# eceo-epfl/ScaleProtoSeg

Measured on AMD Instinct MI355X. Metric: Mpix/s fwd+bwd prototype-distance, Cityscapes 1024x2048, higher is better.
Workload: dtype bf16; 1 GPU; cityscapes_1024x2048_c256_p190_s1; latent_px_per_gpu=2097152, channels=256, prototypes=190, scales=1, classes=19, features_dtype=bf16, parallelism=single

## Files before the change

include/spx_hip.h:

```cpp
#ifndef SPX_HIP_H
#define SPX_HIP_H

#include <stddef.h>
#include <stdint.h>

#ifdef __cplusplus
extern "C" {
#endif

#define SPX_MAX_PANELS 64
#define SPX_ABI_VERSION 17
#define SPX_PRUNE_MAX_K 64

typedef struct spx_plan {
    int32_t num_prototypes;
    int32_t num_classes;
    int32_t num_scales;
    int32_t channels_per_scale;
    int32_t kc;
    int32_t npb;
    int32_t ncb;
    int32_t npanels;
    int32_t panel_ch0[SPX_MAX_PANELS];
    int32_t panel_p0[SPX_MAX_PANELS];
// ... 83 lines not shown
               float* d_logits, void* stream);
int spx_ce_finish(const float* partials, int64_t n_pairs, float* loss, float* count_sum, void* stream);
int spx_shift_labels(const void* labels, int32_t is_int64, int64_t n, int32_t* out, void* stream);

size_t spx_pixel_outer_workspace_bytes(int64_t M, int32_t n1, int32_t n2);
int spx_pixel_outer(const float* a, const float* b, int64_t M, int32_t n1, int32_t n2, float* out, void* workspace, void* stream);

size_t spx_rows_gemm_workspace_bytes(int32_t M, int32_t N, int32_t K, int32_t flags);
int spx_rows_gemm(const float* A, int64_t a_row_stride, int64_t a_k_stride, const float* B, int64_t b_row_stride,
                  int64_t b_k_stride, float* C, int64_t ldc, int32_t M, int32_t N, int32_t K, int32_t flags, const float* E,
                  int64_t lde, void* workspace, void* stream);

size_t spx_group_tail_workspace_bytes(const spx_plan* plan, int32_t B, int32_t HW);
int spx_dist_fwd_group_ws(const spx_plan* plan, const void* x, int32_t x_dtype, int32_t B, int32_t HW,
                          const void* packed_bank, const float* packed_p2, const void* packed_head,
                          const float* Wg, int32_t K2, float* distances, float* activations,
                          float* group_activations, float* logits, const spx_ce* ce, void* workspace,
                          float epsilon, int32_t act_fn, void* stream);
int spx_dist_bwd_group_ce(const spx_plan* plan, const void* x, int32_t x_dtype, int32_t B, int32_t HW,
                          const void* packed_bank, const void* packed_bankT, const float* packed_p2,
                          const void* packed_headT_units, const void* packed_tailT, int32_t K2,
                          const float* group_activations, const float* d_dist, const float* d_act,
                          const spx_ce* ce, const float* d_group_activations, float* d_units, void* dx, void* dx_acc, void* g_out,
                          void* a_out, float epsilon, int32_t act_fn, void* stream);

int spx_group_dense(const float* const* block_ptrs, const int32_t* block_cols, int32_t nblocks, const int32_t* row_block,
                    const int32_t* row_local, const int32_t* col_block, const int32_t* col_local, int32_t U, int32_t P, float* out,
                    void* stream);
int spx_group_dense_bwd(const float* d_out, const int32_t* flat_row, const int32_t* flat_col, int64_t n, int32_t P, float* d_flat,
                        void* stream);
size_t spx_packed_tail_bytes(const spx_plan* plan);
int spx_pack_group_tail(const spx_plan* plan, const float* Wg, int32_t K2, void* packed_tail, void* packed_tailT,
                        void* stream);
int spx_pack_headT_units(const spx_plan* plan, const float* W, void* packed_headT_units, void* stream);
int spx_dist_fwd_group(const spx_plan* plan, const void* x, int32_t x_dtype, int32_t B, int32_t HW,
                       const void* packed_bank, const float* packed_p2, const void* packed_head,
                       const void* packed_tail, int32_t K2,
                       float* distances, float* activations, float* group_activations, float* logits,
                       float epsilon, int32_t act_fn, void* stream);
int spx_dist_bwd_group(const spx_plan* plan, const void* x, int32_t x_dtype, int32_t B, int32_t HW,
                       const void* packed_bank, const void* packed_bankT, const float* packed_p2,
                       const void* packed_headT_units, const void* packed_tailT, int32_t K2,
                       const float* group_activations, const float* d_dist, const float* d_act,
                       const float* d_logits, const float* d_group_activations, float* d_units, void* dx, void* dx_acc, void* g_out,
                       void* a_out, float epsilon, int32_t act_fn, void* stream);
int spx_exp(const float* x, float* y, int64_t n, void* stream);
int spx_exp_bwd(const float* g, const float* y, float* dx, int64_t n, void* stream);

size_t spx_bwd_scratch_bytes(const spx_plan* plan, int32_t B, int32_t HW);
size_t spx_bwd_head_scratch_bytes(const spx_plan* plan, int32_t B, int32_t HW);
size_t spx_bwd_dx_scratch_bytes(const spx_plan* plan, int32_t x_dtype, int32_t B, int32_t HW);

size_t spx_bank_bwd_workspace_bytes(const spx_plan* plan, int32_t B, int32_t HW);
int spx_bank_bwd(const spx_plan* plan, const void* x, int32_t x_dtype, int32_t B, int32_t HW,
                 const float* bank, const void* g_in, const void* a_in, const float* d_logits,
                 float* d_bank, float* d_W, void* workspace, void* stream);

int spx_push_argmin(const float* distances, const int32_t* labels, const float* class_identity,
                    int32_t B, int32_t P, int32_t K, int32_t HW, int32_t void_class, float max_dist,
                    int64_t* indices, float* values, uint64_t* scratch, void* stream);

int spx_dist_push_min(const spx_plan* plan, const void* x, int32_t x_dtype, int32_t B, int32_t HW, const void* packed_bank,
                      const float* packed_p2, const int32_t* labels, int32_t void_class, int32_t K, const uint32_t* proto_key,
                      float max_dist, int64_t* indices, float* values, uint64_t* scratch, void* stream);

int spx_argmin_images(const float* values, int32_t N, int32_t P, int64_t* best, void* stream);

int spx_kld_segment_max(const float* vals, const int32_t* labels, int32_t B, int32_t J, int32_t HW, int32_t W, int32_t K,
                        uint32_t* smax_keys, uint32_t* counts, uint32_t* range_keys, void* stream);
int spx_kld_segment_sumexp(const float* vals, const int32_t* labels, int32_t B, int32_t J, int32_t HW, int32_t W, int32_t K,
                           const uint32_t* smax_keys, uint64_t* ssum_fx, void* stream);
int spx_kld_segment_lse(const uint32_t* smax_keys, const uint64_t* ssum_fx, int32_t n, float* lse, const uint32_t* range_keys,
                        int32_t HW, double* scale, void* stream);
int spx_kld_gram_loss(const int64_t* a_fx, const double* scale, const uint32_t* counts, const uint8_t* pair_ok, int32_t nseg, int32_t K,
                      int32_t J, float* A, float* Cf, double* partials, float* loss, void* stream);
int spx_kld_pair_sums(const float* vals, const int32_t* labels, int32_t B, int32_t J, int32_t HW, int32_t W, int32_t K,
                      const float* lse, const double* scale, int64_t* a_fx, void* stream);
int spx_kld_backward(const float* vals, const int32_t* labels, int32_t B, int32_t J, int32_t HW, int32_t K,
                     const float* lse, const float* A, const float* Cf, const float* cf_scale, float* grad, void* stream);

int spx_upsample_argext(const float* src, int32_t N, int32_t C, int32_t h, int32_t w, int32_t H, int32_t W,
                        int32_t take_max, int64_t* indices, float* values, void* stream);

int spx_eval_accumulate(const float* logits, const int64_t* host_logit_strides, const float* distances,
                        const int64_t* host_dist_strides, const int32_t* proto_class, const void* labels, int32_t label_bytes,
                        int32_t N, int32_t K, int32_t P, int32_t h, int32_t w, int32_t H, int32_t W, int64_t* conf,
                        int64_t* hits, void* stream);
int spx_eval_topk(const float* logits, const int64_t* host_logit_strides, const float* distances, const int64_t* host_dist_strides,
                  const int32_t* proto_class, const void* samples, int32_t sample_bytes, int32_t N, int32_t S, int32_t K,
                  int32_t P, int32_t h, int32_t w, int32_t H, int32_t W, int64_t* topk, int64_t* seen, void* stream);
int spx_eval_check_classes(const int32_t* host_classes, int32_t P, int32_t K);

int spx_prune_argmin(const float* distances, const int32_t* labels, int32_t void_label, int32_t B, int32_t P, int32_t HW,
                     uint64_t* keys, void* stream);
int spx_dist_prune_min(const spx_plan* plan, const void* x, int32_t x_dtype, int32_t B, int32_t HW, const void* packed_bank,
                       const float* packed_p2, const int32_t* labels, int32_t void_label, const uint32_t* proto_key, uint64_t* keys,
                       void* stream);
int spx_prune_footprint(const int32_t* labels, int32_t B, int32_t Hf, int32_t Wf, int32_t H, int32_t W, int32_t P,
                        const uint64_t* keys, const int32_t* target_class, int32_t* label, int32_t* box, void* stream);
int spx_prune_merge(const uint64_t* keys, const int32_t* label, const int32_t* box, int32_t B, int32_t P, int32_t W, int64_t image0,
                    int32_t k, uint64_t* table_key, int64_t* table_image, int32_t* table_label, int32_t* table_box, int32_t* table_cell,
                    void* stream);

#define SPX_REG_ENT 1
#define SPX_REG_CEG 2
#define SPX_REG_SMAX 4
// ... 60 lines not shown
```

scaleprotoseg_amd/_lib.py:

```python
from __future__ import annotations

import ctypes as C
import os
from typing import Optional

import torch

_HERE = os.path.dirname(os.path.abspath(__file__))
LIB_PATH = os.path.join(_HERE, "libspx_hip.so")
SPX_MAX_PANELS = 64
ABI_VERSION = 17


class SpxError(RuntimeError):
    """A libspx_hip.so entry point returned a non-zero status."""


class SpxPlan(C.Structure):
    _fields_ = [
        ("num_prototypes", C.c_int32),
        ("num_classes", C.c_int32),
        ("num_scales", C.c_int32),
        ("channels_per_scale", C.c_int32),
        ("kc", C.c_int32),
# ... 51 lines not shown
    _fields_ = [
        ("vals", C.c_void_p),
        ("labels", C.c_void_p),
        ("slot_scale", C.c_void_p),
        ("B", C.c_int32),
        ("J", C.c_int32),
        ("HW", C.c_int32),
        ("W", C.c_int32),
        ("K", C.c_int32),
        ("mode", C.c_int32),
        ("terms", C.c_int32),
        ("norm_type", C.c_int32),
        ("epsilon", C.c_float),
        ("weights", C.c_float * 3),
    ]


_PP = C.POINTER(SpxPlan)
_PCE = C.POINTER(SpxCe)
_PR = C.POINTER(SpxReg)
_PA = C.POINTER(SpxActLoss)
_V = C.c_void_p
_I = C.c_int32
_F = C.c_float
_PL = C.POINTER(C.c_int64)

SIGNATURES = {
    "spx_version": (C.c_int, []),
    "spx_last_error": (C.c_char_p, []),
    "spx_make_plan": (C.c_int, [_I, _I, _I, _I, C.POINTER(_I), C.POINTER(_I), _PP]),
    "spx_packed_bank_bytes": (C.c_size_t, [_PP]),
    "spx_packed_bankT_bytes": (C.c_size_t, [_PP]),
    "spx_packed_p2_bytes": (C.c_size_t, [_PP]),
    "spx_packed_head_bytes": (C.c_size_t, [_PP]),
    "spx_packed_headT_bytes": (C.c_size_t, [_PP]),
    "spx_pack_bank": (C.c_int, [_PP, _V, _V, _V, _V, _V]),
    "spx_pack_head": (C.c_int, [_PP, _V, _V, _V, _V]),
    "spx_pack_all": (C.c_int, [_PP, _V, _V, _V, _I, _V, _V, _V, _V, _V, _V, _V, _V]),
    "spx_dist_fwd": (C.c_int, [_PP, _V, _I, _I, _I, _V, _V, _V, _V, _V, _V, _F, _I, _V]),
    "spx_dist_bwd": (C.c_int, [_PP, _V, _I, _I, _I, _V, _V, _V, _V, _V, _V, _V, _V, _V, _V, _V, _F, _I, _V]),
    "spx_dist_fwd_cls": (C.c_int, [_PP, _V, _I, _I, _I, _V, _V, _V, _V, _V, _I, _V, _V, _V, _F, _I, _V]),
    "spx_dist_bwd_cls": (C.c_int, [_PP, _V, _I, _I, _I, _V, _V, _V, _V, _V, _V, _I, _V, _V, _V, _V, _V, _V, _V, _F, _I, _V]),
    "spx_group_dense": (C.c_int, [_V, _V, _I, _V, _V, _V, _V, _I, _I, _V, _V]),
    "spx_group_dense_bwd": (C.c_int, [_V, _V, _V, C.c_int64, _I, _V, _V]),
    "spx_packed_tail_bytes": (C.c_size_t, [_PP]),
    "spx_pack_group_tail": (C.c_int, [_PP, _V, _I, _V, _V, _V]),
    "spx_pack_headT_units": (C.c_int, [_PP, _V, _V, _V]),
    "spx_dist_fwd_group": (C.c_int, [_PP, _V, _I, _I, _I, _V, _V, _V, _V, _I, _V, _V, _V, _V, _F, _I, _V]),
    "spx_dist_bwd_group": (C.c_int, [_PP, _V, _I, _I, _I, _V, _V, _V, _V, _V, _I, _V, _V, _V, _V, _V, _V, _V, _V, _V, _V, _F, _I, _V]),
    "spx_bwd_scratch_bytes": (C.c_size_t, [_PP, _I, _I]),
    "spx_bwd_head_scratch_bytes": (C.c_size_t, [_PP, _I, _I]),
    "spx_bwd_dx_scratch_bytes": (C.c_size_t, [_PP, _I, _I, _I]),
    "spx_bank_bwd_workspace_bytes": (C.c_size_t, [_PP, _I, _I]),
    "spx_bank_bwd": (C.c_int, [_PP, _V, _I, _I, _I, _V, _V, _V, _V, _V, _V, _V, _V]),
    "spx_push_argmin": (C.c_int, [_V, _V, _V, _I, _I, _I, _I, _I, _F, _V, _V, _V, _V]),
    "spx_dist_push_min": (C.c_int, [_PP, _V, _I, _I, _I, _V, _V, _V, _I, _I, _V, _F, _V, _V, _V, _V]),
    "spx_argmin_images": (C.c_int, [_V, _I, _I, _V, _V]),
    "spx_kld_segment_max": (C.c_int, [_V, _V, _I, _I, _I, _I, _I, _V, _V, _V, _V]),
    "spx_kld_segment_sumexp": (C.c_int, [_V, _V, _I, _I, _I, _I, _I, _V, _V, _V]),
    "spx_kld_segment_lse": (C.c_int, [_V, _V, _I, _V, _V, _I, _V, _V]),
    "spx_kld_gram_loss": (C.c_int, [_V, _V, _V, _V, _I, _I, _I, _V, _V, _V, _V, _V]),
    "spx_kld_pair_sums": (C.c_int, [_V, _V, _I, _I, _I, _I, _I, _V, _V, _V, _V]),
    "spx_kld_backward": (C.c_int, [_V, _V, _I, _I, _I, _I, _V, _V, _V, _V, _V, _V]),
    "spx_upsample_argext": (C.c_int, [_V, _I, _I, _I, _I, _I, _I, _I, _V, _V, _V]),
    "spx_fwd_split_groups": (C.c_int32, [_PP, _I, _I]),
    "spx_fwd_split_workspace_bytes": (C.c_size_t, [_PP, _I, _I]),
    "spx_dist_fwd_ws": (C.c_int, [_PP, _V, _I, _I, _I, _V, _V, _V, _V, _V, _I, _V, _V, _V, _V, _V, _F, _I, _V]),
    "spx_group_tail_workspace_bytes": (C.c_size_t, [_PP, _I, _I]),
    "spx_dist_fwd_group_ws": (C.c_int, [_PP, _V, _I, _I, _I, _V, _V, _V, _V, _I, _V, _V, _V, _V, _PCE, _V, _F, _I, _V]),
    "spx_dist_bwd_group_ce": (C.c_int, [_PP, _V, _I, _I, _I, _V, _V, _V, _V, _V, _I, _V, _V, _V, _PCE, _V, _V, _V, _V, _V, _V, _F, _I, _V]),
    "spx_exp": (C.c_int, [_V, _V, C.c_int64, _V]),
    "spx_exp_bwd": (C.c_int, [_V, _V, _V, C.c_int64, _V]),
    "spx_pixel_outer_workspace_bytes": (C.c_size_t, [C.c_int64, _I, _I]),
    "spx_pixel_outer": (C.c_int, [_V, _V, C.c_int64, _I, _I, _V, _V, _V]),
    "spx_rows_gemm_workspace_bytes": (C.c_size_t, [_I, _I, _I, _I]),
    "spx_rows_gemm": (C.c_int, [_V, C.c_int64, C.c_int64, _V, C.c_int64, C.c_int64, _V, C.c_int64, _I, _I, _I, _I, _V, C.c_int64, _V, _V]),
    "spx_ce_partials": (C.c_size_t, [_I, _I]),
    "spx_ce_partials_flat": (C.c_size_t, [C.c_int64]),
    "spx_ce_finish": (C.c_int, [_V, C.c_int64, _V, _V, _V]),
    "spx_shift_labels": (C.c_int, [_V, _I, C.c_int64, _V, _V]),
    "spx_dist_fwd_ce": (C.c_int, [_PP, _V, _I, _I, _I, _V, _V, _V, _V, _V, _I, _V, _V, _V, _V, _PCE, _F, _I, _V]),
    "spx_dist_bwd_ce": (C.c_int, [_PP, _V, _I, _I, _I, _V, _V, _V, _V, _V, _V, _I, _V, _V, _V, _PCE, _V, _V, _V, _V, _F, _I, _V]),
    "spx_ce_fwd": (C.c_int, [_V, _V, C.c_int64, _I, _V, _V, _V, _V]),
    "spx_ce_bwd": (C.c_int, [_V, _V, _V, _V, C.c_int64, _I, _V, _V]),
    "spx_eval_accumulate": (C.c_int, [_V, _PL, _V, _PL, _V, _V, _I, _I, _I, _I, _I, _I, _I, _I, _V, _V, _V]),
    "spx_eval_topk": (C.c_int, [_V, _PL, _V, _PL, _V, _V, _I, _I, _I, _I, _I, _I, _I, _I, _I, _V, _V, _V]),
    "spx_eval_check_classes": (C.c_int, [C.POINTER(_I), _I, _I]),
    "spx_prune_argmin": (C.c_int, [_V, _V, _I, _I, _I, _I, _V, _V]),
    "spx_dist_prune_min": (C.c_int, [_PP, _V, _I, _I, _I, _V, _V, _V, _I, _V, _V, _V]),
    "spx_prune_footprint": (C.c_int, [_V, _I, _I, _I, _I, _I, _I, _V, _V, _V, _V, _V]),
    "spx_prune_merge": (C.c_int, [_V, _V, _V, _I, _I, _I, C.c_int64, _I, _V, _V, _V, _V, _V, _V]),
    "spx_reg_workspace_bytes": (C.c_size_t, [_PR]),
    "spx_reg_fwd": (C.c_int, [_PR, _V, _V, _V, _V]),
    "spx_reg_bwd": (C.c_int, [_PR, _V, _V, _V, _V, _V]),
    "spx_actloss_workspace_bytes": (C.c_size_t, [_PA]),
    "spx_actloss_segment_max": (C.c_int, [_PA, _V, _V]),
    "spx_actloss_segment_sums": (C.c_int, [_PA, _V, _V]),
    "spx_actloss_finish": (C.c_int, [_PA, _V, _V, _V, _V]),
    "spx_actloss_backward": (C.c_int, [_PA, _V, _V, _V, _V, _V]),
    "spx_overlap_workspace_bytes": (C.c_size_t, [_I, _I, _I]),
    "spx_overlap_thresholds": (C.c_int, [_V, _PL, _I, _I, _I, _I, _I, _I, C.c_int64, _F, _V, _V, _V]),
    "spx_overlap_accumulate": (C.c_int, [_V, _PL, _V, _V, _I, _V, _I, _I, _I, _I, _I, _I, _I, _I, _V, _V, _V, _V, _V]),
    "spx_push_boxes": (C.c_int, [_V, _PL, _V, _I, _V, _V, _V, _I, _I, _I, _I, _I, _I, _I, _I, _V, _V, _V]),
    "spx_push_merge": (C.c_int, [_V, _V, _V, _I, _I, _I, _I, _I, _I, _V, C.c_int64, _V, _V, _V, _V, _V]),
}

# ... 59 lines not shown
```

scaleprotoseg_amd/csrc/spx_api.hip:

```cpp
#include <stdarg.h>
#include <stdio.h>
#include <string.h>

#include "spx_args.h"

static thread_local char g_err[512] = "";
#ifdef SPX_DIAG
static unsigned long long* g_dbg = nullptr;
static int g_tile_mul_req = 0;
#else
static constexpr unsigned long long* g_dbg = nullptr;
static constexpr int g_tile_mul_req = 0;
#endif

static int gcd_i(int a, int b) { while (b) { const int t = a % b; a = b; b = t; } return a; }
int spx_tile_mul(int tiles_launch, long long plane_bytes) {
    int m = g_tile_mul_req;
    if (m == 0) m = (plane_bytes > 0 && plane_bytes % (1ll << 20) == 0) ? 257 : 1;
    if (m <= 1 || tiles_launch < 4 * m) return 1;
    while (gcd_i(m, tiles_launch) != 1) ++m;
    return m;
}

static int fail(const char* fmt, ...) {
// ... 520 lines not shown
    if (!g || !y || !dx || n < 1 || (n + 255) / 256 > 0x7fffffffLL) return fail("spx_exp_bwd: bad arguments");
    return hip_status(spx_launch_exp(nullptr, g, y, dx, n, (hipStream_t)stream), "spx_exp_bwd");
}

int spx_group_dense(const float* const* block_ptrs, const int32_t* block_cols, int32_t nblocks, const int32_t* row_block,
                    const int32_t* row_local, const int32_t* col_block, const int32_t* col_local, int32_t U, int32_t P, float* out,
                    void* stream) {
    if (!block_ptrs || !block_cols || !row_block || !row_local || !col_block || !col_local || !out) return fail("spx_group_dense: NULL buffer");
    if (nblocks < 1 || nblocks > SPX_GROUP_BLOCKS_MAX) return fail("spx_group_dense: %d blocks (1..%d)", nblocks, SPX_GROUP_BLOCKS_MAX);
    if (U < 1 || P < 1 || (long long)U * P > 0x7fffffffLL) return fail("spx_group_dense: bad sizes (U=%d P=%d)", U, P);
    SpxGroupDenseArgs a{};
    for (int j = 0; j < nblocks; ++j) {
        if (!block_ptrs[j] || block_cols[j] < 1) return fail("spx_group_dense: block %d is empty", j);
        a.ptrs[j] = block_ptrs[j];
        a.ncols[j] = block_cols[j];
    }
    a.row_block = row_block; a.row_local = row_local; a.col_block = col_block; a.col_local = col_local;
    a.U = U; a.P = P; a.out = out;
    return hip_status(spx_launch_group_dense(a, (hipStream_t)stream), "spx_group_dense");
}
int spx_group_dense_bwd(const float* d_out, const int32_t* flat_row, const int32_t* flat_col, int64_t n, int32_t P, float* d_flat,
                        void* stream) {
    if (!d_out || !flat_row || !flat_col || !d_flat) return fail("spx_group_dense_bwd: NULL buffer");
    if (n < 1 || P < 1 || (n + 255) / 256 > 0x7fffffffLL) return fail("spx_group_dense_bwd: bad sizes");
    return hip_status(spx_launch_group_dense_bwd(d_out, flat_row, flat_col, n, P, d_flat, (hipStream_t)stream), "spx_group_dense_bwd");
}

int spx_ce_fwd(const float* logits, const int32_t* labels, int64_t M, int32_t K, float* lse, int32_t* pred, float* partials,
               void* stream) {
    if (!logits || !labels || !lse || !partials) return fail("spx_ce_fwd: NULL buffer");
    if (M < 1 || K < 1 || (M + 255) / 256 > 0x7fffffffLL) return fail("spx_ce_fwd: bad sizes (M=%lld K=%d)", (long long)M, K);
    return hip_status(spx_launch_ce_fwd(logits, labels, M, K, lse, pred, partials, (hipStream_t)stream), "spx_ce_fwd");
}
int spx_ce_finish(const float* partials, int64_t n_pairs, float* loss, float* count_sum, void* stream) {
    if (!partials || !loss || !count_sum || n_pairs < 1) return fail("spx_ce_finish: bad arguments");
    return hip_status(spx_launch_ce_finish(partials, n_pairs, loss, count_sum, (hipStream_t)stream), "spx_ce_finish");
}
int spx_shift_labels(const void* labels, int32_t is_int64, int64_t n, int32_t* out, void* stream) {
    if (!labels || !out || n < 1 || (n + 255) / 256 > 0x7fffffffLL) return fail("spx_shift_labels: bad arguments");
    return hip_status(spx_launch_shift_labels(labels, is_int64, n, out, (hipStream_t)stream), "spx_shift_labels");
}
int spx_ce_bwd(const float* logits, const float* lse, const int32_t* labels, const float* coef, int64_t M, int32_t K,
               float* d_logits, void* stream) {
    if (!logits || !lse || !labels || !coef || !d_logits) return fail("spx_ce_bwd: NULL buffer");
    if (M < 1 || K < 1 || (M * K + 255) / 256 > 0x7fffffffLL) return fail("spx_ce_bwd: bad sizes (M=%lld K=%d)", (long long)M, K);
    return hip_status(spx_launch_ce_bwd(logits, lse, labels, coef, M, K, d_logits, (hipStream_t)stream), "spx_ce_bwd");
}

size_t spx_bank_bwd_workspace_bytes(const spx_plan* pl, int32_t B, int32_t HW) {
    const int nsplit = spx_bank_bwd_nsplit(*pl, B, HW);
    return spx_bank_bwd_ws_floats(*pl, nsplit) * sizeof(float);
}

int spx_bank_bwd(const spx_plan* pl, const void* x, int32_t x_dtype, int32_t B, int32_t HW, const float* bank,
                 const void* g_in, const void* a_in, const float* d_logits, float* d_bank, float* d_W,
                 void* workspace, void* stream) {
    if (check_plan(pl)) return 1;
    if (!x || !bank || !workspace) return fail("spx_bank_bwd: NULL operand");
    if (x_dtype != 0 && x_dtype != 1) return fail("spx_bank_bwd: x_dtype %d", x_dtype);
    if (d_bank && !g_in) return fail("spx_bank_bwd: d_bank requested without G");
    if (d_W && !a_in) return fail("spx_bank_bwd: d_W requested without the head-gradient scratch of spx_dist_bwd");
    if (d_W && pl->ncb > 1 && !d_logits) return fail("spx_bank_bwd: d_W of a head wider than 32 rows needs d_logits");
    if (pl->channels_per_scale > 256) return fail("spx_bank_bwd: Cs %d > 256 not supported", pl->channels_per_scale);
    SpxBankBwdArgs a;
    a.plan = *pl;
    a.x = x;
    a.bank = bank;
    a.g_in = (const uint16_t*)g_in;
    a.a_in = (const uint16_t*)a_in;
    a.d_logits = d_logits;
    a.d_bank = d_bank;
    a.d_W = d_W;
    a.workspace = (float*)workspace;
    a.B = B;
    a.HW = HW;
    a.nsplit = spx_bank_bwd_nsplit(*pl, B, HW);
    return hip_status(spx_launch_bank_bwd(a, x_dtype, (hipStream_t)stream), "spx_bank_bwd");
}

int spx_push_argmin(const float* distances, const int32_t* labels, const float* class_identity, int32_t B, int32_t P,
                    int32_t K, int32_t HW, int32_t void_class, float max_dist, int64_t* indices, float* values,
                    uint64_t* scratch, void* stream) {
    if (!distances || !labels || !class_identity || !indices || !values || !scratch)
        return fail("spx_push_argmin: NULL buffer");
    if (B < 1 || P < 1 || K < 1 || HW < 1) return fail("spx_push_argmin: empty input");
    if (K > 160) return fail("spx_push_argmin: num_classes %d > 160", K);
    if (P > 65535 || B > 65535) return fail("spx_push_argmin: grid too large");
    return hip_status(spx_launch_push_argmin(distances, labels, class_identity, B, P, K, HW, void_class, max_dist,
                                             indices, values, scratch, (hipStream_t)stream),
                      "spx_push_argmin");
}

int spx_prune_argmin(const float* distances, const int32_t* labels, int32_t void_label, int32_t B, int32_t P, int32_t HW,
                     uint64_t* keys, void* stream) {
    if (!distances || !labels || !keys) return fail("spx_prune_argmin: NULL buffer");
    if (B < 1 || P < 1 || HW < 1) return fail("spx_prune_argmin: empty input (B=%d P=%d HW=%d)", B, P, HW);
    if (P > 0x7FFF8 || B > 65535) return fail("spx_prune_argmin: grid too large (B=%d P=%d)", B, P);
    return hip_status(spx_launch_prune_argmin(distances, labels, void_label, B, P, HW, keys, (hipStream_t)stream), "spx_prune_argmin");
}

int spx_prune_footprint(const int32_t* labels, int32_t B, int32_t Hf, int32_t Wf, int32_t H, int32_t W, int32_t P,
                        const uint64_t* keys, const int32_t* target_class, int32_t* label, int32_t* box, void* stream) {
    if (!labels || !keys || !target_class || !label || !box) return fail("spx_prune_footprint: NULL buffer");
    if (B < 1 || P < 1 || Hf < 1 || Wf < 1 || H < 1 || W < 1)
        return fail("spx_prune_footprint: empty input (B=%d P=%d Hf=%d Wf=%d H=%d W=%d)", B, P, Hf, Wf, H, W);
    if (B > 65535 || P > 0x7FFFFFFF / 4) return fail("spx_prune_footprint: grid too large (B=%d P=%d)", B, P);
// ... 317 lines not shown
```

scaleprotoseg_amd/csrc/spx_args.h:

```cpp
#pragma once
#include "spx_common.h"
#include <type_traits>

struct SpxFwdArgs {
    spx_plan plan;
    const void* x;
    const char* packed_bank;
    const float* p2;
    const char* packed_head;
    float* dist;
    float* act;
    float* logits;
    int B, HW, vec_ok;
    int tile_first, tiles_launch;
    int tile_mul;
    int dist_vec;
    const int32_t* labels;
    const uint32_t* proto_key;
    float* cls_dist;
    int J;
    unsigned long long* push_keys;
    float push_max;
    int push_void, push_K;
    int push_prune;
// ... 33 lines not shown
    int ngroups;
    int32_t group_first[SPX_MAX_PANELS + 1];
    const int32_t* ce_labels;
    const float* ce_logits;
    const float* ce_lse;
    const float* ce_coef;
    float* ce_dlogits_out;
    void* dx;
    float* dx_acc;
    uint16_t* g_out;
    uint16_t* a_out;
    int B, HW, vec_ok;
    int tile_first, tiles_launch;
    int tile_mul;
    float eps;
    int act_fn;
    unsigned long long* dbg;
};
struct SpxBankBwdArgs {
    spx_plan plan;
    const void* x;
    const float* bank;
    const uint16_t* g_in;
    const uint16_t* a_in;
    const float* d_logits;
    float* d_bank;
    float* d_W;
    float* workspace;
    int B, HW, vec_ok, nsplit;
    int ci_first, nci_launch;
    int slab_first, nslabs;
};
__host__ __device__ inline uint32_t spx_blob_slot(int r, int h, int s2) {
    return (uint32_t)(((r >> 2) * 8 + (r & 3) + 4 * h + 8 * s2) & 63);
}

inline int spx_x_stage_mode(int HW) { return HW < 8 ? 0 : (HW % 8 == 0 ? 1 : 2); }
template <typename F>
static inline void spx_dispatch_x(int x_dtype, int vm, F f) {
    auto with_vm = [&](auto xf32) {
        if (vm == 2) f(xf32, std::integral_constant<int, 2>{});
        else if (vm) f(xf32, std::integral_constant<int, 1>{});
        else f(xf32, std::integral_constant<int, 0>{});
    };
    if (x_dtype == 1) with_vm(std::true_type{});
    else with_vm(std::false_type{});
}

int spx_tile_mul(int tiles_launch, long long plane_bytes);
hipError_t spx_launch_fwd(const SpxFwdArgs& a, int x_dtype, hipStream_t s);
hipError_t spx_launch_bwd(const SpxBwdArgs& a, int x_dtype, hipStream_t s);
hipError_t spx_launch_bank_bwd(const SpxBankBwdArgs& a, int x_dtype, hipStream_t s);
int spx_bank_bwd_nsplit(const spx_plan& pl, int B, int HW);
size_t spx_bwd_scratch_elems(const spx_plan& pl, int B, int HW);
size_t spx_bank_bwd_ws_floats(const spx_plan& pl, int nsplit);
hipError_t spx_launch_pack_bank(const spx_plan& pl, const float* bank, void* pb, void* pbT, float* p2, hipStream_t s);
hipError_t spx_launch_pack_head(const spx_plan& pl, const float* W, void* ph, void* phT, hipStream_t s);
hipError_t spx_launch_pack_tail(const spx_plan& pl, const float* Wg, int K2, void* pt, void* ptT, hipStream_t s);
hipError_t spx_launch_pack_headT_units(const spx_plan& pl, const float* W, void* phT, hipStream_t s);
struct SpxPackAllArgs {
    spx_plan plan;
    const float* bank;
    const float* W;
    const float* Wg;
    int K2, headT_units;
    void *packed_bank, *packed_bankT;
    float* p2;
    void *packed_head, *packed_headT, *packed_tail, *packed_tailT;
    int nb_bank, nb_head, nb_headT;
};
hipError_t spx_launch_pack_all(SpxPackAllArgs a, hipStream_t s);
hipError_t spx_launch_ce_finish(const float* partials, long long n, float* loss, float* aux, hipStream_t s);
hipError_t spx_launch_shift_labels(const void* in, int is64, long long n, int32_t* out, hipStream_t s);
#define SPX_GROUP_BLOCKS_MAX 192
struct SpxGroupDenseArgs {
    const float* ptrs[SPX_GROUP_BLOCKS_MAX];
    int ncols[SPX_GROUP_BLOCKS_MAX];
    const int32_t *row_block, *row_local, *col_block, *col_local;
    int U, P;
    float* out;
};
hipError_t spx_launch_group_dense(const SpxGroupDenseArgs& a, hipStream_t s);
hipError_t spx_launch_group_dense_bwd(const float* d_out, const int32_t* rows, const int32_t* cols, long long n, int P, float* d_flat,
                                      hipStream_t s);
hipError_t spx_launch_push_argmin(const float* dist, const int32_t* labels, const float* ident, int B, int P, int K,
                                  int HW, int void_class, float max_dist, int64_t* idx, float* val,
                                  uint64_t* scratch, hipStream_t s);
hipError_t spx_launch_argmin_images(const float* values, int N, int P, int64_t* best, hipStream_t s);
hipError_t spx_launch_push_merge(const int64_t* indices, const float* values, const void* x, int x_dtype, int B, int P, int C, int HW,
                                 int Cs, const int32_t* proto_scale, long long image0, float* best_value, int64_t* best_image,
                                 int64_t* best_flat, float* best_patch, hipStream_t s);
hipError_t spx_launch_upsample_argext(const float* src, int N, int C, int h, int w, int H, int W, int take_max,
                                      int64_t* idx, float* val, hipStream_t s);
hipError_t spx_launch_eval_accumulate(const float* logits, const long long* lst, const float* dist, const long long* dst,
                                      const int32_t* pcls, const void* labels, int label_bytes, int N, int K, int P, int h, int w,
                                      int H, int W, unsigned long long* conf, unsigned long long* hits, hipStream_t s);
hipError_t spx_launch_eval_topk(const float* logits, const long long* lst, const float* dist, const long long* dst,
                                const int32_t* pcls, const void* samples, int sample_bytes, int N, int S, int K, int P, int h,
                                int w, int H, int W, unsigned long long* topk, unsigned long long* seen, hipStream_t s);
hipError_t spx_launch_sum_groups(const float* parts, size_t n, int groups, float* out, hipStream_t s);
int spx_split_groups(const spx_plan& pl, int B, int HW, int32_t* group_first);
hipError_t spx_launch_group_tail(const float* parts, int groups, long long M, int U, const float* Wg, int K2, float* gact,
                                 float* logits, const int32_t* labels, float* lse, int32_t* pred, float* partials, hipStream_t s);
hipError_t spx_launch_push_finalize(const uint64_t* scratch, int n, int64_t* idx, float* val, hipStream_t s);
hipError_t spx_launch_prune_argmin(const float* dist, const int32_t* labels, int void_label, int B, int P, int HW,
                                   uint64_t* keys, hipStream_t s);
// ... 51 lines not shown
```

scaleprotoseg_amd/csrc/spx_bank.hip:

```cpp
#include "spx_args.h"
#include "spx_common.h"
#include <type_traits>

#define SPX_BK_THREADS 512
#define SPX_BANK_PIPE 1
#define SPX_BANK_STAGGER 1
__host__ __device__ constexpr int spx_bk_row(int cpx) { return 2 * cpx + 16; }

__host__ __device__ inline int spx_bk_wstride(const spx_plan& pl) {
    return ((pl.channels_per_scale + 31) / 32) * 32 + pl.ncb * 32 + 32;
}
static void spx_bank_parts(const spx_plan& pl, int B, int HW, int& nci, int& nci_vec, int& slabs_vec, int& slabs_tail) {
    nci = 2 * ((HW + SPX_TILE_PX - 1) / SPX_TILE_PX);
    nci_vec = HW >= 8 ? nci : 0;
    long long cap = 256 / pl.npanels;
    if (cap < 1) cap = 1;
    const long long cv = (long long)B * nci_vec, ct = (long long)B * (nci - nci_vec);
    slabs_vec = (int)(cv < cap ? cv : cap);
    slabs_tail = (int)(ct < cap ? ct : cap);
}
int spx_bank_bwd_nsplit(const spx_plan& pl, int B, int HW) {
    int nci, nci_vec, sv, st;
    spx_bank_parts(pl, B, HW, nci, nci_vec, sv, st);
    return sv + st;
}
size_t spx_bank_bwd_ws_floats(const spx_plan& pl, int nsplit) {
    return (size_t)nsplit * pl.npanels * pl.npb * 32 * spx_bk_wstride(pl);
}
template <int NPB, int NCB, bool DO_P, bool DO_W, int CPX>
__host__ __device__ constexpr int spx_bk_buf_bytes() {
    constexpr int fb = (CPX / 32) * NPB * 2 * 1024;
    return (DO_P ? fb + 256 * spx_bk_row(CPX) : 0) + (DO_W ? 2 * fb + 2 * NCB * 32 * spx_bk_row(CPX) : 0);
}
template <int NPB, int NCB, bool DO_P, bool DO_W, int CPX>
__host__ __device__ constexpr int spx_bk_lds_bytes() {
    constexpr int red = (2 * 3 * 2 * 1024 + 2 * 3 * 64) * 4;
    constexpr int n = (CPX == 32 ? 2 : 1) * spx_bk_buf_bytes<NPB, NCB, DO_P, DO_W, CPX>();
    return (n > red ? n : red) + 16;
}

template <int NPB, int NCB, bool XF32, int VM, bool DO_P, bool DO_W, bool KSPLIT, int CPX>
__global__ __launch_bounds__(SPX_BK_THREADS, 2) void spx_bank_bwd_kernel(const SpxBankBwdArgs a) {
    constexpr bool VEC = VM != 0, RAG = VM == 2;
    constexpr int SPX_BK_PX = CPX, SPX_BK_ROW = spx_bk_row(CPX);
    constexpr int NW1 = CPX / 32;
    constexpr bool PIPE = CPX == 32;
    static_assert(!(PIPE && KSPLIT), "the k-step split needs four pixel k-steps per chunk");
    extern __shared__ __attribute__((aligned(16))) char smem[];
    const spx_plan& pl = a.plan;
    const int tid = threadIdx.x, lane = tid & 63;
    const int wave = __builtin_amdgcn_readfirstlane(tid >> 6);
    const int r = lane & 31, h = lane >> 5;
    const int q = blockIdx.y, split = blockIdx.x;
    const int Cs = pl.channels_per_scale, K = pl.num_classes;
// ... 390 lines not shown
#pragma unroll
                for (int c = 0; c < 3; ++c) {
#pragma unroll
                    for (int t = 0; t < 2; ++t)
#pragma unroll
                        for (int reg = 0; reg < 16; ++reg)
                            accp[i][t][reg] += red[(((half * 3 + c) * 2 + t) * 16 + reg) * 64 + lane];
                    csum[i] += redc[(half * 3 + c) * 64 + lane];
                }
            }
        }
    }

    const int ws = spx_bk_wstride(pl);
    float* slab = a.workspace + ((size_t)(a.slab_first + split) * pl.npanels + q) * rows * ws;
    const float sinv_acc = have_e ? __builtin_amdgcn_ldexpf(1.0f, -e_acc) : 0.0f;
    if (want_p && (!ksplit || cpair == 0)) {
#pragma unroll
        for (int i = 0; i < PH; ++i) {
            const int pb = pb0 + i;
#pragma unroll
            for (int t = 0; t < 2; ++t) {
                const int chb = ksplit ? t : 2 * cpair + t;
                if (chb < nchb) {
#pragma unroll
                    for (int reg = 0; reg < 16; ++reg)
                        slab[(size_t)(pb * 32 + acc_row(reg, h)) * ws + chb * 32 + r] = accp[i][t][reg] * sinv_acc;
                }
            }
            if (ksplit ? cpair == 0 : cpair == cs_owner(i)) {
                const float s = csum[i] + __shfl_xor(csum[i], 32);
                if (h == 0) slab[(size_t)(pb * 32 + r) * ws + nchb * 32 + NCB * 32] = s * sinv_acc;
            }
        }
    }
    if (want_w && w_role) {
#pragma unroll
        for (int cb = 0; cb < NCB; ++cb) {
#pragma unroll
            for (int reg = 0; reg < 16; ++reg)
                slab[(size_t)(wave * 32 + acc_row(reg, h)) * ws + nchb * 32 + cb * 32 + r] = accw[cb][reg];
        }
    }
}

#define SPX_BD_GSLOTS 4
#define SPX_BD_XSLOTS 3
#define SPX_BD_XUNIT (256 * 128)
template <int NPB>
__host__ __device__ constexpr int spx_bd_lds_bytes() {
    return SPX_BD_GSLOTS * NPB * 2 * 1024 + SPX_BD_XSLOTS * SPX_BD_XUNIT + (SPX_BD_GSLOTS + 1) * 1024;
}

template <int NPB>
__global__ __launch_bounds__(SPX_BK_THREADS, 2) void spx_bank_dma_kernel(const SpxBankBwdArgs a) {
    extern __shared__ __attribute__((aligned(16))) char smem[];
    const spx_plan& pl = a.plan;
    const int tid = threadIdx.x, lane = tid & 63;
    const int wave = __builtin_amdgcn_readfirstlane(tid >> 6);
    const int r = lane & 31, h = lane >> 5;
    const int q = blockIdx.y, split = blockIdx.x;
    const int Cs = pl.channels_per_scale;
    const int C = pl.num_scales * Cs;
    const int nchb = (Cs + 31) / 32;
    constexpr int rows = NPB * 32;
    constexpr int GB = NPB * 2 * 1024;
    constexpr int NGP = NPB * 2 + 1;
    constexpr int PWG = (NGP + 7) / 8;
    constexpr int PW = PWG + 2;
    char* const gring = smem;
    char* const xring = smem + SPX_BD_GSLOTS * GB;
    char* const epad = xring + SPX_BD_XSLOTS * SPX_BD_XUNIT;
    char* const trash = epad + SPX_BD_GSLOTS * 1024;
    const int ch0 = pl.panel_ch0[q];
    const int tiles_per_img = (a.HW + SPX_TILE_PX - 1) / SPX_TILE_PX;
    const size_t ntiles = (size_t)a.B * tiles_per_img;
    const int nui = a.nci_launch;
    const long long total = (long long)a.B * nui;
    const long long cstep = a.nslabs;
    const long long u_begin = split;
    const int n_units = u_begin < total ? (int)((total - u_begin + cstep - 1) / cstep) : 0;
    const int n_steps = 2 * n_units;
    const size_t blob_total = (size_t)pl.npanels * ntiles * 4 * NPB * 2 * 1024;
    const int32_t* const gexp = (const int32_t*)((const char*)a.g_in + spx_gexp_offset(blob_total)) + (size_t)q * ntiles;

    const int cpair = wave & 3;
    constexpr int PH = NPB / 2;
    const int pb0 = (wave >> 2) * PH;
    const int cs_first = wave >> 2;
    auto cs_owner = [&](int i) { return i == 0 ? cs_first : i + 1; };
    f32x16 accp[PH][2];
    float csum[PH];
    int e_acc = 0;
    bool have_e = false;
#pragma unroll
    for (int i = 0; i < PH; ++i) {
        csum[i] = 0.0f;
#pragma unroll
        for (int t = 0; t < 2; ++t)
#pragma unroll
            for (int e = 0; e < 16; ++e) accp[i][t][e] = 0.0f;
    }
    for (int o = tid * 16; o < spx_bd_lds_bytes<NPB>(); o += SPX_BK_THREADS * 16) *(u32x4*)(smem + o) = u32x4{0u, 0u, 0u, 0u};
    __syncthreads();

    auto dma = [&](const char* base, uint32_t vo, char* dst) {
        const uint64_t ba = (uint64_t)base;
        u32x4 rs;
        rs[0] = __builtin_amdgcn_readfirstlane((uint32_t)ba);
        rs[1] = __builtin_amdgcn_readfirstlane((uint32_t)(ba >> 32) & 0xffffu);
        rs[2] = 0x80000000u;
        rs[3] = 0x00020000u;
        const uint32_t la = __builtin_amdgcn_readfirstlane((uint32_t)(uintptr_t)(__attribute__((address_space(3))) char*)dst);
        uint32_t keep;
        asm volatile("s_mov_b32 %0, m0\n\ts_mov_b32 m0, %1\n\ts_nop 0\n\tbuffer_load_dwordx4 %2, %3, 0 offen lds\n\ts_mov_b32 m0, %0"
                     : "=&s"(keep) : "s"(la), "v"(vo), "s"(rs) : "memory");
    };
    struct Cursor {
        int k, b, ui;
    };
    const int step_b = (int)(cstep / nui), step_ui = (int)(cstep - (long long)step_b * nui);
    auto advance = [&](Cursor& c) {
        ++c.k;
        if (c.k < n_units) {
            c.b += step_b;
            c.ui += step_ui;
            if (c.ui >= nui) {
                c.ui -= nui;
                ++c.b;
            }
        }
    };
    Cursor cg, cx;
    cg.k = cx.k = 0;
    cg.b = cx.b = (int)(u_begin / nui);
    cg.ui = cx.ui = (int)(u_begin - (long long)cg.b * nui);
    auto issue_g = [&](int gs, int e) {
        const size_t tile_g = (size_t)cg.b * tiles_per_img + (cg.ui >> 1);
        const char* const gsrc = (const char*)a.g_in + ((((size_t)q * ntiles + tile_g) * 4 + 2 * (cg.ui & 1) + e) * NPB * 2) * 1024;
#pragma unroll
        for (int i = 0; i < PWG; ++i) {
            const int p = wave + 8 * i;
            const bool is_g = p < NPB * 2, is_e = p == NPB * 2;
            dma(is_g ? gsrc + (size_t)p * 1024 : (const char*)(gexp + tile_g),
                is_g ? (uint32_t)lane * 16u : ((is_e && lane == 0) ? 0u : SPX_OOB),
                is_g ? gring + gs * GB + p * 1024 : (is_e ? epad + gs * 1024 : trash));
        }
    };
    auto issue_x = [&](int xs, int e) {
#pragma unroll
        for (int i = 0; i < 2; ++i) {
            const int p = 16 * e + wave + 8 * i;
            const int row = 8 * p + (lane >> 3);
            const int px = cx.ui * 64 + 8 * ((lane & 7) ^ ((row >> 1) & 7));
            dma((const char*)a.x + ((size_t)cx.b * C + ch0 + 8 * p) * a.HW * 2,
                (row < Cs && px + 8 <= a.HW) ? ((uint32_t)(lane >> 3) * (uint32_t)a.HW + (uint32_t)px) * 2u : SPX_OOB,
                xring + xs * SPX_BD_XUNIT + p * 1024);
// ... 174 lines not shown
    if (is_p) {
        a.d_bank[(size_t)p * Cs + col] = 2.0f * (a.bank[(size_t)p * Cs + col] * ct - st);
    } else {
        const size_t ntl = (size_t)a.B * ((a.HW + SPX_TILE_PX - 1) / SPX_TILE_PX);
        const size_t off = pl.ncb == 1 ? spx_dw_partial_bytes(pl.npanels, ntl, pl.npb, K) : spx_ablob_scale_offset(ntl * pl.npanels * 4 * pl.npb * 2 * 1024);
        a.d_W[(size_t)(col - Cs) * P + p] = *(const float*)((const char*)a.a_in + off) * st;
    }
}

__global__ __launch_bounds__(256) void spx_dw_reduce_kernel(const SpxBankBwdArgs a) {
    const spx_plan& pl = a.plan;
    const int j = blockIdx.x, q = blockIdx.y;
    const int K = pl.num_classes, NPB = pl.npb;
    const int nchb = (pl.channels_per_scale + 31) / 32;
    const int rows = NPB * 32, ws = spx_bk_wstride(pl);
    const long long ntiles = (long long)a.B * ((a.HW + SPX_TILE_PX - 1) / SPX_TILE_PX);
    const int nvb = (pl.panel_np[q] + 31) >> 5;
    const int nvec = nvb * K * 8;
    const size_t tstride = (size_t)NPB * K * 32;
    const float* const base = (const float*)a.a_in + (size_t)q * ntiles * tstride;
    float* const slab = a.workspace + ((size_t)j * pl.npanels + q) * rows * ws;
    for (int v = threadIdx.x; v < nvec; v += 256) {
        f32x4 s[8];
#pragma unroll
        for (int u = 0; u < 8; ++u) s[u] = f32x4{0.f, 0.f, 0.f, 0.f};
        long long t = j;
        for (; t + 7ll * a.nsplit < ntiles; t += 8ll * a.nsplit) {
#pragma unroll
            for (int u = 0; u < 8; ++u) s[u] += *(const f32x4*)(base + (size_t)(t + (long long)u * a.nsplit) * tstride + (size_t)v * 4);
        }
        for (int u = 0; t < ntiles; t += a.nsplit, ++u) s[u] += *(const f32x4*)(base + (size_t)t * tstride + (size_t)v * 4);
        const f32x4 tot = ((s[0] + s[1]) + (s[2] + s[3])) + ((s[4] + s[5]) + (s[6] + s[7]));
        const int pb = v / (K * 8), rem = v - pb * (K * 8), cls = rem >> 3, p4 = rem & 7;
#pragma unroll
        for (int e = 0; e < 4; ++e) slab[(size_t)(pb * 32 + p4 * 4 + e) * ws + nchb * 32 + cls] = tot[e];
    }
}

template <int NPB, int NCB, bool DO_P, bool DO_W, bool KSPLIT>
static hipError_t launch_bank_k(const SpxBankBwdArgs& a, int x_dtype, dim3 grid, hipStream_t s) {
    constexpr int CPX = (SPX_BANK_PIPE && !KSPLIT && NPB == 6 && NCB == 1 && 2 * spx_bk_buf_bytes<NPB, NCB, DO_P, DO_W, 32>() <= SPX_LDS_LIMIT) ? 32 : 64;
    constexpr size_t lds = (size_t)spx_bk_lds_bytes<NPB, NCB, DO_P, DO_W, CPX>();
    static_assert(lds <= SPX_LDS_LIMIT, "bank kernel LDS");
    spx_dispatch_x(x_dtype, a.vec_ok, [&](auto xf32, auto vm) {
        hipLaunchKernelGGL((spx_bank_bwd_kernel<NPB, NCB, decltype(xf32)::value, decltype(vm)::value, DO_P, DO_W, KSPLIT, CPX>), grid, dim3(SPX_BK_THREADS), lds, s, a);
    });
    return hipGetLastError();
}
template <int NPB, int NCB, bool DO_P, bool DO_W>
static hipError_t launch_bank_pw(const SpxBankBwdArgs& a, int x_dtype, dim3 grid, hipStream_t s) {
    if (DO_P && a.plan.channels_per_scale <= 64) return launch_bank_k<NPB, NCB, DO_P, DO_W, true>(a, x_dtype, grid, s);
    return launch_bank_k<NPB, NCB, DO_P, DO_W, false>(a, x_dtype, grid, s);
}
template <int NPB, int NCB>
static hipError_t launch_bank_x(const SpxBankBwdArgs& a, int x_dtype, dim3 grid, hipStream_t s) {
    if constexpr (NCB == 1) {
        if (!a.d_bank) return hipSuccess;
        if (x_dtype == 0 && a.vec_ok == 1 && a.HW % 64 == 0 && a.plan.channels_per_scale > 64) {
            constexpr size_t lds = (size_t)spx_bd_lds_bytes<NPB>();
            static_assert(lds <= SPX_LDS_LIMIT, "bank kernel LDS");
            hipLaunchKernelGGL((spx_bank_dma_kernel<NPB>), grid, dim3(SPX_BK_THREADS), lds, s, a);
            return hipGetLastError();
        }
        return launch_bank_pw<NPB, NCB, true, false>(a, x_dtype, grid, s);
    } else if constexpr (NCB < 5) {
        if (!a.d_bank) return launch_bank_pw<NPB, NCB, false, true>(a, x_dtype, grid, s);
        return launch_bank_pw<NPB, NCB, true, true>(a, x_dtype, grid, s);
    } else {
        hipError_t e = hipSuccess;
        if (a.d_bank) e = launch_bank_pw<NPB, NCB, true, false>(a, x_dtype, grid, s);
        if (e == hipSuccess && a.d_W) e = launch_bank_pw<NPB, NCB, false, true>(a, x_dtype, grid, s);
        return e;
    }
}

static hipError_t spx_launch_bank_part(const SpxBankBwdArgs& a, int x_dtype, hipStream_t s) {
    const spx_plan& pl = a.plan;
    dim3 grid((unsigned)a.nslabs, (unsigned)pl.npanels);
    if (pl.ncb == 1)
        return pl.npb == 2 ? launch_bank_x<2, 1>(a, x_dtype, grid, s) : pl.npb == 4 ? launch_bank_x<4, 1>(a, x_dtype, grid, s) : launch_bank_x<6, 1>(a, x_dtype, grid, s);
    if (pl.ncb == 2)
        return pl.npb == 2 ? launch_bank_x<2, 2>(a, x_dtype, grid, s) : pl.npb == 4 ? launch_bank_x<4, 2>(a, x_dtype, grid, s) : launch_bank_x<6, 2>(a, x_dtype, grid, s);
    return pl.npb == 2 ? launch_bank_x<2, 5>(a, x_dtype, grid, s) : pl.npb == 4 ? launch_bank_x<4, 5>(a, x_dtype, grid, s) : launch_bank_x<6, 5>(a, x_dtype, grid, s);
}

hipError_t spx_launch_bank_bwd(const SpxBankBwdArgs& a0, int x_dtype, hipStream_t s) {
    SpxBankBwdArgs a = a0;
    const spx_plan& pl = a.plan;
    const int rows = pl.npb * 32;
    int nci, nci_vec, sv, st;
    spx_bank_parts(pl, a.B, a.HW, nci, nci_vec, sv, st);
    a.nsplit = sv + st;
    hipError_t e = hipSuccess;
    if (sv > 0) {
        a.vec_ok = a.HW % 8 == 0 ? 1 : 2; a.ci_first = 0; a.nci_launch = nci_vec; a.slab_first = 0; a.nslabs = sv;
        e = spx_launch_bank_part(a, x_dtype, s);
    }
    if (e == hipSuccess && st > 0) {
        a.vec_ok = 0; a.ci_first = nci_vec; a.nci_launch = nci - nci_vec; a.slab_first = sv; a.nslabs = st;
        e = spx_launch_bank_part(a, x_dtype, s);
    }
    if (e != hipSuccess) return e;
    if (pl.ncb == 1 && a.d_W) {
        hipLaunchKernelGGL(spx_dw_reduce_kernel, dim3((unsigned)a.nsplit, (unsigned)pl.npanels), dim3(256), 0, s, a);
        if ((e = hipGetLastError()) != hipSuccess) return e;
    }
    const long long n = (long long)pl.npanels * rows * (pl.channels_per_scale + pl.num_classes);
    hipLaunchKernelGGL(spx_bank_reduce_kernel, dim3((unsigned)((n + SPX_RED_ELEMS - 1) / SPX_RED_ELEMS)),
                       dim3(SPX_RED_ELEMS * SPX_RED_PARTS), 0, s, a);
    return hipGetLastError();
}
```

Before: 805.4 Mpix/s.

## Fold dW partial reduction into extra waves of the bank DMA kernel

```diff
diff --git a/include/spx_hip.h b/include/spx_hip.h
--- a/include/spx_hip.h
+++ b/include/spx_hip.h
@@ -159,6 +159,7 @@
 size_t spx_bwd_dx_scratch_bytes(const spx_plan* plan, int32_t x_dtype, int32_t B, int32_t HW);
 
 size_t spx_bank_bwd_workspace_bytes(const spx_plan* plan, int32_t B, int32_t HW);
+int spx_bank_bwd_dw_folded(const spx_plan* plan, int32_t x_dtype, int32_t HW, int32_t want_d_bank, int32_t want_d_W);
 int spx_bank_bwd(const spx_plan* plan, const void* x, int32_t x_dtype, int32_t B, int32_t HW,
                  const float* bank, const void* g_in, const void* a_in, const float* d_logits,
                  float* d_bank, float* d_W, void* workspace, void* stream);
diff --git a/scaleprotoseg_amd/_lib.py b/scaleprotoseg_amd/_lib.py
--- a/scaleprotoseg_amd/_lib.py
+++ b/scaleprotoseg_amd/_lib.py
@@ -127,6 +127,7 @@
     "spx_bwd_head_scratch_bytes": (C.c_size_t, [_PP, _I, _I]),
     "spx_bwd_dx_scratch_bytes": (C.c_size_t, [_PP, _I, _I, _I]),
     "spx_bank_bwd_workspace_bytes": (C.c_size_t, [_PP, _I, _I]),
+    "spx_bank_bwd_dw_folded": (C.c_int, [_PP, _I, _I, _I, _I]),
     "spx_bank_bwd": (C.c_int, [_PP, _V, _I, _I, _I, _V, _V, _V, _V, _V, _V, _V, _V]),
     "spx_push_argmin": (C.c_int, [_V, _V, _V, _I, _I, _I, _I, _I, _F, _V, _V, _V, _V]),
     "spx_dist_push_min": (C.c_int, [_PP, _V, _I, _I, _I, _V, _V, _V, _I, _I, _V, _F, _V, _V, _V, _V]),
diff --git a/scaleprotoseg_amd/csrc/spx_api.hip b/scaleprotoseg_amd/csrc/spx_api.hip
--- a/scaleprotoseg_amd/csrc/spx_api.hip
+++ b/scaleprotoseg_amd/csrc/spx_api.hip
@@ -596,6 +596,11 @@
     return spx_bank_bwd_ws_floats(*pl, nsplit) * sizeof(float);
 }
 
+int spx_bank_bwd_dw_folded(const spx_plan* pl, int32_t x_dtype, int32_t HW, int32_t want_d_bank, int32_t want_d_W) {
+    if (check_plan(pl)) return 0;
+    return spx_bank_bwd_folds_dw(*pl, x_dtype, HW, want_d_bank != 0, want_d_W != 0) ? 1 : 0;
+}
+
 int spx_bank_bwd(const spx_plan* pl, const void* x, int32_t x_dtype, int32_t B, int32_t HW, const float* bank,
                  const void* g_in, const void* a_in, const float* d_logits, float* d_bank, float* d_W,
                  void* workspace, void* stream) {
diff --git a/scaleprotoseg_amd/csrc/spx_args.h b/scaleprotoseg_amd/csrc/spx_args.h
--- a/scaleprotoseg_amd/csrc/spx_args.h
+++ b/scaleprotoseg_amd/csrc/spx_args.h
@@ -109,6 +109,7 @@
 hipError_t spx_launch_bwd(const SpxBwdArgs& a, int x_dtype, hipStream_t s);
 hipError_t spx_launch_bank_bwd(const SpxBankBwdArgs& a, int x_dtype, hipStream_t s);
 int spx_bank_bwd_nsplit(const spx_plan& pl, int B, int HW);
+bool spx_bank_bwd_folds_dw(const spx_plan& pl, int x_dtype, int HW, bool want_bank, bool want_w);
 size_t spx_bwd_scratch_elems(const spx_plan& pl, int B, int HW);
 size_t spx_bank_bwd_ws_floats(const spx_plan& pl, int nsplit);
 hipError_t spx_launch_pack_bank(const spx_plan& pl, const float* bank, void* pb, void* pbT, float* p2, hipStream_t s);
diff --git a/scaleprotoseg_amd/csrc/spx_bank.hip b/scaleprotoseg_amd/csrc/spx_bank.hip
--- a/scaleprotoseg_amd/csrc/spx_bank.hip
+++ b/scaleprotoseg_amd/csrc/spx_bank.hip
@@ -1,5 +1,6 @@
 #include "spx_args.h"
 #include "spx_common.h"
+#include <cstdlib>
 #include <type_traits>
 
 #define SPX_BK_THREADS 512
@@ -496,8 +497,66 @@
     return SPX_BD_GSLOTS * NPB * 2 * 1024 + SPX_BD_XSLOTS * SPX_BD_XUNIT + (SPX_BD_GSLOTS + 1) * 1024;
 }
 
-template <int NPB>
-__global__ __launch_bounds__(SPX_BK_THREADS, 2) void spx_bank_dma_kernel(const SpxBankBwdArgs a) {
+template <int RW>
+__device__ __forceinline__ void spx_dw_fold(const SpxBankBwdArgs& a, int q, int j, int rt, int n_steps) {
+    const spx_plan& pl = a.plan;
+    const int K = pl.num_classes, NPB = pl.npb;
+    const int nchb = (pl.channels_per_scale + 31) / 32;
+    const int rows = NPB * 32, ws = spx_bk_wstride(pl);
+    const long long ntiles = (long long)a.B * ((a.HW + SPX_TILE_PX - 1) / SPX_TILE_PX);
+    const int nvb = (pl.panel_np[q] + 31) >> 5;
+    const int nvec = nvb * K * 8;
+    const size_t tstride = (size_t)NPB * K * 32;
+    const float* const base = (const float*)a.a_in + (size_t)q * ntiles * tstride;
+    float* const slab = a.workspace + ((size_t)j * pl.npanels + q) * rows * ws;
+    const int nt = j < ntiles ? (int)((ntiles - j + a.nsplit - 1) / a.nsplit) : 0;
+    const int nfull = nt >> 3, rem = nt & 7;
+    const int ngrp = nfull + (rem ? 1 : 0);
+    const int npass = (nvec + 64 * RW - 1) / (64 * RW);
+    const int nticks = npass * (ngrp + 1);
+    f32x4 s[8], ld[8];
+#pragma unroll
+    for (int u = 0; u < 8; ++u) s[u] = f32x4{0.f, 0.f, 0.f, 0.f};
+    int pass = 0, g = 0, done = 0, due = 0;
+    for (int st = 0; st <= n_steps; ++st) {
+        int todo = nticks - done;
+        if (st < n_steps) {
+            __builtin_amdgcn_s_barrier();
+            due += nticks;
+            todo = due / n_steps;
+            due -= todo * n_steps;
+        }
+        for (; todo > 0; --todo, ++done) {
+            const int v = rt + pass * 64 * RW;
+            const bool on = v < nvec;
+            if (g > 0) {
+                const int cnt = g - 1 < nfull ? 8 : rem;
+#pragma unroll
+                for (int u = 0; u < 8; ++u) s[u] += u < cnt ? ld[u] : f32x4{0.f, 0.f, 0.f, 0.f};
+            }
+            if (g < ngrp) {
+                const float* const src = base + (size_t)(on ? v : nvec - 1) * 4;
+#pragma unroll
+                for (int u = 0; u < 8; ++u) ld[u] = *(const f32x4*)(src + (size_t)(j + (long long)min(8 * g + u, nt - 1) * a.nsplit) * tstride);
+                ++g;
+            } else {
+                if (on) {
+                    const f32x4 tot = ((s[0] + s[1]) + (s[2] + s[3])) + ((s[4] + s[5]) + (s[6] + s[7]));
+                    const int pb = v / (K * 8), r8 = v - pb * (K * 8), cls = r8 >> 3, p4 = r8 & 7;
+#pragma unroll
+                    for (int e = 0; e < 4; ++e) slab[(size_t)(pb * 32 + p4 * 4 + e) * ws + nchb * 32 + cls] = tot[e];
+                }
+#pragma unroll
+                for (int u = 0; u < 8; ++u) s[u] = f32x4{0.f, 0.f, 0.f, 0.f};
+                g = 0;
+                ++pass;
+            }
+        }
+    }
+}
+
+template <int NPB, int RW>
+__global__ __launch_bounds__(SPX_BK_THREADS + 64 * RW, RW ? 1 : 2) void spx_bank_dma_kernel(const SpxBankBwdArgs a) {
     extern __shared__ __attribute__((aligned(16))) char smem[];
     const spx_plan& pl = a.plan;
     const int tid = threadIdx.x, lane = tid & 63;
@@ -545,8 +604,14 @@
 #pragma unroll
             for (int e = 0; e < 16; ++e) accp[i][t][e] = 0.0f;
     }
-    for (int o = tid * 16; o < spx_bd_lds_bytes<NPB>(); o += SPX_BK_THREADS * 16) *(u32x4*)(smem + o) = u32x4{0u, 0u, 0u, 0u};
+    for (int o = tid * 16; o < spx_bd_lds_bytes<NPB>(); o += (SPX_BK_THREADS + 64 * RW) * 16) *(u32x4*)(smem + o) = u32x4{0u, 0u, 0u, 0u};
     __syncthreads();
+    if constexpr (RW > 0) {
+        if (wave >= SPX_BK_THREADS / 64) {
+            spx_dw_fold<RW>(a, q, a.slab_first + split, tid - SPX_BK_THREADS, n_steps);
+            return;
+        }
+    }
 
     auto dma = [&](const char* base, uint32_t vo, char* dst) {
         const uint64_t ba = (uint64_t)base;
@@ -827,14 +892,26 @@
     if (DO_P && a.plan.channels_per_scale <= 64) return launch_bank_k<NPB, NCB, DO_P, DO_W, true>(a, x_dtype, grid, s);
     return launch_bank_k<NPB, NCB, DO_P, DO_W, false>(a, x_dtype, grid, s);
 }
+static bool spx_bank_dma_runs(const spx_plan& pl, int x_dtype, int HW) {
+    return x_dtype == 0 && HW % 64 == 0 && pl.channels_per_scale > 64;
+}
+#ifndef SPX_BD_RED_WAVES
+#define SPX_BD_RED_WAVES 2
+#endif
+bool spx_bank_bwd_folds_dw(const spx_plan& pl, int x_dtype, int HW, bool want_bank, bool want_w) {
+    if (pl.ncb != 1 || !want_bank || !want_w || !spx_bank_dma_runs(pl, x_dtype, HW)) return false;
+    const char* const e = getenv("SPX_BANK_DW_FOLD");
+    return !(e && e[0] == '0');
+}
 template <int NPB, int NCB>
-static hipError_t launch_bank_x(const SpxBankBwdArgs& a, int x_dtype, dim3 grid, hipStream_t s) {
+static hipError_t launch_bank_x(const SpxBankBwdArgs& a, int x_dtype, dim3 grid, bool fold_dw, hipStream_t s) {
     if constexpr (NCB == 1) {
         if (!a.d_bank) return hipSuccess;
-        if (x_dtype == 0 && a.vec_ok == 1 && a.HW % 64 == 0 && a.plan.channels_per_scale > 64) {
+        if (a.vec_ok == 1 && spx_bank_dma_runs(a.plan, x_dtype, a.HW)) {
             constexpr size_t lds = (size_t)spx_bd_lds_bytes<NPB>();
             static_assert(lds <= SPX_LDS_LIMIT, "bank kernel LDS");
-            hipLaunchKernelGGL((spx_bank_dma_kernel<NPB>), grid, dim3(SPX_BK_THREADS), lds, s, a);
+            if (fold_dw) hipLaunchKernelGGL((spx_bank_dma_kernel<NPB, SPX_BD_RED_WAVES>), grid, dim3(SPX_BK_THREADS + 64 * SPX_BD_RED_WAVES), lds, s, a);
+            else hipLaunchKernelGGL((spx_bank_dma_kernel<NPB, 0>), grid, dim3(SPX_BK_THREADS), lds, s, a);
             return hipGetLastError();
         }
         return launch_bank_pw<NPB, NCB, true, false>(a, x_dtype, grid, s);
@@ -849,14 +926,14 @@
     }
 }
 
-static hipError_t spx_launch_bank_part(const SpxBankBwdArgs& a, int x_dtype, hipStream_t s) {
+static hipError_t spx_launch_bank_part(const SpxBankBwdArgs& a, int x_dtype, bool fold_dw, hipStream_t s) {
     const spx_plan& pl = a.plan;
     dim3 grid((unsigned)a.nslabs, (unsigned)pl.npanels);
     if (pl.ncb == 1)
-        return pl.npb == 2 ? launch_bank_x<2, 1>(a, x_dtype, grid, s) : pl.npb == 4 ? launch_bank_x<4, 1>(a, x_dtype, grid, s) : launch_bank_x<6, 1>(a, x_dtype, grid, s);
+        return pl.npb == 2 ? launch_bank_x<2, 1>(a, x_dtype, grid, fold_dw, s) : pl.npb == 4 ? launch_bank_x<4, 1>(a, x_dtype, grid, fold_dw, s) : launch_bank_x<6, 1>(a, x_dtype, grid, fold_dw, s);
     if (pl.ncb == 2)
-        return pl.npb == 2 ? launch_bank_x<2, 2>(a, x_dtype, grid, s) : pl.npb == 4 ? launch_bank_x<4, 2>(a, x_dtype, grid, s) : launch_bank_x<6, 2>(a, x_dtype, grid, s);
-    return pl.npb == 2 ? launch_bank_x<2, 5>(a, x_dtype, grid, s) : pl.npb == 4 ? launch_bank_x<4, 5>(a, x_dtype, grid, s) : launch_bank_x<6, 5>(a, x_dtype, grid, s);
+        return pl.npb == 2 ? launch_bank_x<2, 2>(a, x_dtype, grid, fold_dw, s) : pl.npb == 4 ? launch_bank_x<4, 2>(a, x_dtype, grid, fold_dw, s) : launch_bank_x<6, 2>(a, x_dtype, grid, fold_dw, s);
+    return pl.npb == 2 ? launch_bank_x<2, 5>(a, x_dtype, grid, fold_dw, s) : pl.npb == 4 ? launch_bank_x<4, 5>(a, x_dtype, grid, fold_dw, s) : launch_bank_x<6, 5>(a, x_dtype, grid, fold_dw, s);
 }
 
 hipError_t spx_launch_bank_bwd(const SpxBankBwdArgs& a0, int x_dtype, hipStream_t s) {
@@ -866,17 +943,18 @@
     int nci, nci_vec, sv, st;
     spx_bank_parts(pl, a.B, a.HW, nci, nci_vec, sv, st);
     a.nsplit = sv + st;
+    const bool fold_dw = spx_bank_bwd_folds_dw(pl, x_dtype, a.HW, a.d_bank != nullptr, a.d_W != nullptr);
     hipError_t e = hipSuccess;
     if (sv > 0) {
         a.vec_ok = a.HW % 8 == 0 ? 1 : 2; a.ci_first = 0; a.nci_launch = nci_vec; a.slab_first = 0; a.nslabs = sv;
-        e = spx_launch_bank_part(a, x_dtype, s);
+        e = spx_launch_bank_part(a, x_dtype, fold_dw, s);
     }
     if (e == hipSuccess && st > 0) {
         a.vec_ok = 0; a.ci_first = nci_vec; a.nci_launch = nci - nci_vec; a.slab_first = sv; a.nslabs = st;
-        e = spx_launch_bank_part(a, x_dtype, s);
+        e = spx_launch_bank_part(a, x_dtype, fold_dw, s);
     }
     if (e != hipSuccess) return e;
-    if (pl.ncb == 1 && a.d_W) {
+    if (pl.ncb == 1 && a.d_W && !fold_dw) {
         hipLaunchKernelGGL(spx_dw_reduce_kernel, dim3((unsigned)a.nsplit, (unsigned)pl.npanels), dim3(256), 0, s, a);
         if ((e = hipGetLastError()) != hipSuccess) return e;
     }
```

Result: no change. 804.1 Mpix/s (-0.2%).
